# icdm-adteam/MoCoPCI

Measured on AMD Instinct MI355X. Metric: interpolated frames/sec, higher is better.
Workload: dtype f32 (fused MLP layers: fp32 products as 6 bf16-MFMA partials of an exact 3-way split, fp32 accumulate; index paths exact f32)

## Files before the change

mocopci_amd/csrc/knn_cosine.hip:

```cpp
#include "common.h"
#include "topk.h"

namespace {

typedef mcp_key u64;
typedef float f32x16 __attribute__((ext_vector_type(16)));
#define KEY_INF MCP_KEY_INF
constexpr int K = 16, QS = 16, CHK = 4, RT = 32, WAVES = 4;

__device__ __forceinline__ int chan_of(int r, int h) { return (r & 3) + 8 * (r >> 2) + 4 * h; }

template <int C>
__global__ __launch_bounds__(256) void normalize_rows_kernel(long long rows_a, const float *__restrict__ xa, float *__restrict__ ya,
                                                             long long rows_b, const float *__restrict__ xb, float *__restrict__ yb) {
    constexpr int RW = C <= 64 ? 64 : (C == 128 ? 32 : 16), S = C + 1, V = RW * C / 4;
    __shared__ float tile[4][RW * S];
    __shared__ float den[4][RW];
    const int lane = threadIdx.x & 63, wave = threadIdx.x >> 6;
    float *t = tile[wave];
    const long long ta = (rows_a + RW - 1) / RW, tb = (rows_b + RW - 1) / RW;
    for (long long g = (long long)blockIdx.x * 4 + wave; g < ta + tb; g += (long long)gridDim.x * 4) {
        const bool second = g >= ta;
        const float *x = second ? xb : xa;
        float *y = second ? yb : ya;
        const long long rows = second ? rows_b : rows_a, r0 = (second ? g - ta : g) * RW;
        const int live = (int)min((long long)RW, rows - r0);
        const float4 *src = reinterpret_cast<const float4 *>(x + r0 * C);
        __builtin_amdgcn_wave_barrier();
        for (int e = lane; e < V; e += 64) {
            const int row = (e * 4) / C, col = (e * 4) % C;
            if (row < live) {
                const float4 v = src[e];
                float *d = t + row * S + col;
                d[0] = v.x; d[1] = v.y; d[2] = v.z; d[3] = v.w;
            }
        }
        __builtin_amdgcn_wave_barrier();
        if (lane < live) {
            const float *xr = t + lane * S;
            float s = 0.f;
            for (int j = 0; j < C; ++j) s = s + xr[j] * xr[j];
            den[wave][lane] = sqrtf(s + 1e-8f);
        }
        __builtin_amdgcn_wave_barrier();
        float4 *dst = reinterpret_cast<float4 *>(y + r0 * C);
        for (int e = lane; e < V; e += 64) {
            const int row = (e * 4) / C, col = (e * 4) % C;
            if (row < live) {
                const float *d = t + row * S + col;
                const float dn = den[wave][row];
                dst[e] = make_float4(d[0] / dn, d[1] / dn, d[2] / dn, d[3] / dn);
            }
        }
    }
}

template <int C>
void launch_normalize(long long rows_a, const float *xa, float *ya, long long rows_b, const float *xb, float *yb, hipStream_t s) {
    constexpr int RW = C <= 64 ? 64 : (C == 128 ? 32 : 16);
    const long long tiles = (rows_a + RW - 1) / RW + (rows_b + RW - 1) / RW, blocks = (tiles + 3) / 4;
    hipLaunchKernelGGL(normalize_rows_kernel<C>, dim3((unsigned)min(blocks, 4096LL)), dim3(256), 0, s, rows_a, xa, ya, rows_b, xb, yb);
}

template <int C>
__global__ __launch_bounds__(64 * WAVES) void knn_cosine_kernel(int q, int n, int kout, const float *__restrict__ nq,
                                                                const float *__restrict__ nr, int *__restrict__ idx,
                                                                float *__restrict__ dist) {
    constexpr int S = C + 1;
    constexpr int PER_THREAD = RT * C / (64 * WAVES);
    extern __shared__ __attribute__((aligned(16))) float smem[];
    float *tiles = smem;
    const int tid = threadIdx.x, lane = tid & 63, wave = tid >> 6, h = lane >> 5, col = lane & 31;
    uint2(*queue)[64] = reinterpret_cast<uint2(*)[64]>(smem + 2 * RT * S) + (size_t)wave * QS;

    const int b = blockIdx.y;
    const int qi = blockIdx.x * (32 * WAVES) + wave * 32 + col;
    const bool live = qi < q;
    const float *qrow = nq + ((size_t)b * q + (live ? qi : 0)) * C;
    float bq[C / 2];
#pragma unroll
    for (int s = 0; s < C / 2; ++s) bq[s] = qrow[2 * s + h];
    nr += (size_t)b * n * C;

    u64 a[K];
#pragma unroll
    for (int j = 0; j < K; ++j) a[j] = KEY_INF;
    float tau = INFINITY;
    int cnt = 0;
    auto flush = [&]() {
        mcp_flush_queue<K, QS>(a, queue, lane, cnt);
        tau = mcp_tau_of(a[K - 1]);
        cnt = 0;
    };

    const int ntiles = (n + RT - 1) / RT;
    float pre[PER_THREAD];
    auto fetch = [&](int t) {
#pragma unroll
        for (int u = 0; u < PER_THREAD; ++u) {
            const int e = tid + u * 64 * WAVES, row = e / C, cc = e % C;
            const int gr = t * RT + row;
            pre[u] = gr < n ? nr[(size_t)gr * C + cc] : 0.f;
        }
    };
    auto stash = [&](int buf) {
#pragma unroll
        for (int u = 0; u < PER_THREAD; ++u) {
            const int e = tid + u * 64 * WAVES, row = e / C, cc = e % C;
            tiles[buf * RT * S + row * S + cc] = pre[u];
        }
    };
    fetch(0);
    stash(0);
    for (int t = 0; t < ntiles; ++t) {
        const int cur = t & 1;
        if (t + 1 < ntiles) fetch(t + 1);
        __syncthreads();
        const float *ta = tiles + cur * RT * S + col * S + h;
        f32x16 acc;
#pragma unroll
        for (int r = 0; r < 16; ++r) acc[r] = 0.f;
#pragma unroll
        for (int s = 0; s < C / 2; ++s) acc = __builtin_amdgcn_mfma_f32_32x32x2f32(ta[2 * s], bq[s], acc, 0, 0, 0);
        const int base = t * RT;
#pragma unroll
        for (int r0 = 0; r0 < 16; r0 += CHK) {
#pragma unroll
            for (int r = r0; r < r0 + CHK; ++r) {
                const int ri = base + chan_of(r, h);
                const float d = 1.0f - acc[r];
                if (ri < n && d < tau) {
                    queue[cnt][lane] = make_uint2(__float_as_uint(d), (uint32_t)ri);
                    ++cnt;
                }
            }
            if (__builtin_amdgcn_ballot_w64(cnt > QS - CHK)) flush();
        }
        if (t + 1 < ntiles) stash(cur ^ 1);
    }
    flush();
    u64 o[K];
#pragma unroll
    for (int j = 0; j < K; ++j) {
        const uint32_t lo = __shfl_xor(mcp_key_lo(a[j]), 32), hi = __shfl_xor(mcp_key_hi(a[j]), 32);
        o[j] = mcp_key_words(hi, lo);
    }
    mcp_merge_sorted<K, K>(a, o);
    if (!live || h) return;
    int *oi = idx + ((size_t)b * q + qi) * kout;
    float *od = dist ? dist + ((size_t)b * q + qi) * kout : nullptr;
    mcp_store_list<K>(a, kout, oi, od);
}

template <int C, int RS>
__global__ __launch_bounds__(64 * RS) void knn_cosine_split_kernel(int q, int n, int kout, const float *__restrict__ nq,
                                                                   const float *__restrict__ nr, int *__restrict__ idx,
                                                                   float *__restrict__ dist) {
    constexpr int CH = C / 32;
    extern __shared__ __attribute__((aligned(16))) float smem[];
    const int tid = threadIdx.x, lane = tid & 63, wave = tid >> 6, h = lane >> 5, col = lane & 31;
    uint2(*queue)[64] = reinterpret_cast<uint2(*)[64]>(smem) + (size_t)wave * QS;

    const int b = blockIdx.y;
    const int qi = blockIdx.x * 32 + col;
    const bool live = qi < q;
    const float *qrow = nq + ((size_t)b * q + (live ? qi : 0)) * C;
    constexpr bool QL = C > 128;
    float bq[QL ? 1 : C / 2];
    float *ql = smem + (size_t)RS * QS * 64 * 2;
    if (QL) {
        for (int i = wave; i < C / 2; i += RS) ql[i * 64 + lane] = qrow[2 * i + h];
        __syncthreads();
    } else {
#pragma unroll
        for (int j = 0; j < (QL ? 0 : C / 4); ++j) {
            const float4 v = reinterpret_cast<const float4 *>(qrow)[j];
            bq[QL ? 0 : 2 * j] = h ? v.y : v.x;
            bq[QL ? 0 : 2 * j + 1] = h ? v.w : v.z;
        }
    }
    nr += (size_t)b * n * C;

    u64 a[K];
#pragma unroll
    for (int j = 0; j < K; ++j) a[j] = KEY_INF;
    float tau = INFINITY;
    int cnt = 0;
    auto flush = [&]() {
        mcp_flush_queue<K, QS>(a, queue, lane, cnt);
        tau = mcp_tau_of(a[K - 1]);
        cnt = 0;
    };

    const int ntiles = (n + RT - 1) / RT;
    const int mine = wave < ntiles ? (ntiles - wave + RS - 1) / RS : 0;
    auto load = [&](int t, int c, float4 (&v)[8]) {
        const int row = min(t * RT + col, n - 1);
        const float4 *p = reinterpret_cast<const float4 *>(nr + (size_t)row * C + c * 32);
#pragma unroll
        for (int j = 0; j < 8; ++j) v[j] = p[j];
    };
    f32x16 acc;
    auto mfma16 = [&](int c, const float4 (&v)[8]) {
#pragma unroll
        for (int j = 0; j < 8; ++j) {
            const float q0 = QL ? ql[(c * 16 + 2 * j) * 64 + lane] : bq[QL ? 0 : c * 16 + 2 * j];
            const float q1 = QL ? ql[(c * 16 + 2 * j + 1) * 64 + lane] : bq[QL ? 0 : c * 16 + 2 * j + 1];
            acc = __builtin_amdgcn_mfma_f32_32x32x2f32(h ? v[j].y : v[j].x, q0, acc, 0, 0, 0);
            acc = __builtin_amdgcn_mfma_f32_32x32x2f32(h ? v[j].w : v[j].z, q1, acc, 0, 0, 0);
        }
    };
    float4 va[8], vb[8];
    if (mine > 0) load(wave, 0, va);
    for (int ti = 0; ti < mine; ++ti) {
        const int t = wave + ti * RS;
#pragma unroll
        for (int r = 0; r < 16; ++r) acc[r] = 0.f;
#pragma unroll
        for (int c = 0; c < CH; c += 2) {
            load(t, c + 1, vb);
            mfma16(c, va);
            if (c + 2 < CH) load(t, c + 2, va);
            else if (ti + 1 < mine) load(t + RS, 0, va);
            mfma16(c + 1, vb);
        }
        const int base = t * RT;
#pragma unroll
        for (int r0 = 0; r0 < 16; r0 += CHK) {
#pragma unroll
            for (int r = r0; r < r0 + CHK; ++r) {
                const int ri = base + chan_of(r, h);
                const float d = 1.0f - acc[r];
                if (ri < n && d < tau) {
                    queue[cnt][lane] = make_uint2(__float_as_uint(d), (uint32_t)ri);
                    ++cnt;
                }
            }
            if (__builtin_amdgcn_ballot_w64(cnt > QS - CHK)) flush();
        }
    }
    flush();
    u64 o[K];
#pragma unroll
    for (int j = 0; j < K; ++j) {
        const uint32_t lo = __shfl_xor(mcp_key_lo(a[j]), 32), hi = __shfl_xor(mcp_key_hi(a[j]), 32);
        o[j] = mcp_key_words(hi, lo);
    }
    mcp_merge_sorted<K, K>(a, o);
    __syncthreads();
    if (wave > 0 && h == 0) {
#pragma unroll
        for (int j = 0; j < K; ++j) queue[j][col] = make_uint2(mcp_key_lo(a[j]), mcp_key_hi(a[j]));
    }
    __syncthreads();
    if (wave != 0 || h) return;
    for (int w = 1; w < RS; ++w) {
        uint2(*other)[64] = reinterpret_cast<uint2(*)[64]>(smem) + (size_t)w * QS;
#pragma unroll
        for (int j = 0; j < K; ++j) {
            const uint2 e = other[j][col];
            o[j] = mcp_key_words(e.y, e.x);
        }
        mcp_merge_sorted<K, K>(a, o);
    }
    if (!live) return;
    int *oi = idx + ((size_t)b * q + qi) * kout;
    float *od = dist ? dist + ((size_t)b * q + qi) * kout : nullptr;
    mcp_store_list<K>(a, kout, oi, od);
}

template <int C, int RS>
int launch_cosine_split(int b, int q, int n, int k, const float *nq, const float *nr, int *idx, float *dist, hipStream_t s) {
    static_assert(K == QS && (C / 32) % 2 == 0, "the partial lists reuse the queues; chunks are consumed in pairs");
    const size_t lds = (size_t)RS * QS * 64 * sizeof(uint2) + (C > 128 ? (size_t)(C / 2) * 64 * sizeof(float) : 0);
    auto kern = knn_cosine_split_kernel<C, RS>;
    static McpPerDeviceOnce attr_once;
    if (attr_once.need()) {
        { const hipError_t attr_e_ = hipFuncSetAttribute(reinterpret_cast<const void *>(kern), hipFuncAttributeMaxDynamicSharedMemorySize, 160 * 1024); if (attr_e_ != hipSuccess) return (int)attr_e_; }
        attr_once.done();
    }
    hipLaunchKernelGGL(kern, dim3(mcp_divup(q, 32), b), dim3(64 * RS), lds, s, q, n, k, nq, nr, idx, dist);
    return mcp_launch_status();
}

template <int C>
int launch_cosine_auto(int b, int q, int n, int k, const float *nq, const float *nr, int *idx, float *dist, hipStream_t s) {
    const long long groups = (long long)b * ((q + 31) / 32);
    const int tiles = (n + RT - 1) / RT;
    if (groups * 2 >= 2048 || tiles < 4) return launch_cosine_split<C, 2>(b, q, n, k, nq, nr, idx, dist, s);
    if (groups * 4 >= 2048 || tiles < 8) return launch_cosine_split<C, 4>(b, q, n, k, nq, nr, idx, dist, s);
    return launch_cosine_split<C, 8>(b, q, n, k, nq, nr, idx, dist, s);
}

template <int C>
int launch_cosine(int b, int q, int n, int k, const float *nq, const float *nr, int *idx, float *dist, hipStream_t s) {
    const size_t lds = (size_t)2 * RT * (C + 1) * sizeof(float) + (size_t)WAVES * QS * 64 * sizeof(uint2);
    auto kern = knn_cosine_kernel<C>;
    static McpPerDeviceOnce attr_once;
    if (attr_once.need()) {
        { const hipError_t attr_e_ = hipFuncSetAttribute(reinterpret_cast<const void *>(kern), hipFuncAttributeMaxDynamicSharedMemorySize, 160 * 1024); if (attr_e_ != hipSuccess) return (int)attr_e_; }
        attr_once.done();
    }
    hipLaunchKernelGGL(kern, dim3(mcp_divup(q, 32 * WAVES), b), dim3(64 * WAVES), lds, s, q, n, k, nq, nr, idx, dist);
    return mcp_launch_status();
}

}

#ifdef MCP_AB
static int g_cosine_use_old = 0;
extern "C" __attribute__((visibility("default"))) void mcp_knn_cosine_use_old(int on) { g_cosine_use_old = on; }
#endif

MCP_EXPORT int mcp_knn_cosine(int b, int q, int n, int c, int k, const float *qfeat, const float *rfeat, int *idx, float *dist,
                              float *workspace, mcp_stream_t stream) {
    MCP_CHECK_ARGS(b > 0 && q > 0 && n > 0 && c > 0 && k > 0 && qfeat && rfeat && idx && workspace);
    if (k > K || (c != 64 && c != 128 && c != 256)) return MCP_ERR_UNSUPPORTED;
    if ((((uintptr_t)qfeat) | ((uintptr_t)rfeat) | ((uintptr_t)workspace)) & 15) return MCP_ERR_BAD_ARG;
    hipStream_t s = (hipStream_t)stream;
    float *nq = workspace, *nr = workspace + (size_t)b * q * c;
    mcp_prof_begin(MCP_KERNEL_KNN_COSINE, s);
    const long long rq = (long long)b * q, rr = (long long)b * n;
    if (c == 64) launch_normalize<64>(rq, qfeat, nq, rr, rfeat, nr, s);
    else if (c == 128) launch_normalize<128>(rq, qfeat, nq, rr, rfeat, nr, s);
    else launch_normalize<256>(rq, qfeat, nq, rr, rfeat, nr, s);
    int rc = mcp_launch_status();
    if (rc == MCP_OK) {
#ifdef MCP_AB
        if (g_cosine_use_old)
            rc = c == 64    ? launch_cosine<64>(b, q, n, k, nq, nr, idx, dist, s)
                 : c == 128 ? launch_cosine<128>(b, q, n, k, nq, nr, idx, dist, s)
                            : launch_cosine<256>(b, q, n, k, nq, nr, idx, dist, s);
        else
#endif
        rc = c == 64    ? launch_cosine_auto<64>(b, q, n, k, nq, nr, idx, dist, s)
             : c == 128 ? launch_cosine_auto<128>(b, q, n, k, nq, nr, idx, dist, s)
                        : launch_cosine_auto<256>(b, q, n, k, nq, nr, idx, dist, s);
    }
    mcp_prof_end(MCP_KERNEL_KNN_COSINE, s);
    return rc;
}
```

Before: 3672.

## Add tiled cosine KNN kernel sharing reference tiles across query waves

Adds a new cosine KNN kernel in which several query waves (QG) share LDS-staged reference tiles, split into 64-channel chunks and double-buffered with register prefetch. Reference rows are split across RP wave partitions whose partial top-k lists are merged by a binary tree through LDS. The default auto path now launches this kernel with an XCD-aware unit mapping, and the previous split kernel stays available under A/B flags. The intent is to cut redundant global reads of reference features and improve latency hiding. In exchange it adds block-wide syncs per chunk and an LDS merge stage, and lowers the number of reference partitions, which may reduce parallelism on small batches.

```diff
diff --git a/mocopci_amd/csrc/knn_cosine.hip b/mocopci_amd/csrc/knn_cosine.hip
--- a/mocopci_amd/csrc/knn_cosine.hip
+++ b/mocopci_amd/csrc/knn_cosine.hip
@@ -284,12 +284,180 @@
 }
 
 template <int C>
-int launch_cosine_auto(int b, int q, int n, int k, const float *nq, const float *nr, int *idx, float *dist, hipStream_t s) {
+int launch_cosine_split_auto(int b, int q, int n, int k, const float *nq, const float *nr, int *idx, float *dist, hipStream_t s) {
     const long long groups = (long long)b * ((q + 31) / 32);
     const int tiles = (n + RT - 1) / RT;
     if (groups * 2 >= 2048 || tiles < 4) return launch_cosine_split<C, 2>(b, q, n, k, nq, nr, idx, dist, s);
     if (groups * 4 >= 2048 || tiles < 8) return launch_cosine_split<C, 4>(b, q, n, k, nq, nr, idx, dist, s);
     return launch_cosine_split<C, 8>(b, q, n, k, nq, nr, idx, dist, s);
+}
+
+template <int C, int QG, int RP>
+__global__ __launch_bounds__(64 * QG * RP) void knn_cosine_tiles_kernel(int nb, int q, int n, int kout, const float *__restrict__ nq,
+                                                                        const float *__restrict__ nr, int *__restrict__ idx,
+                                                                        float *__restrict__ dist) {
+    constexpr int CW = 64, S = CW + 1, NCH = C / CW;
+    constexpr int WV = QG * RP, PT = 64 * QG;
+    constexpr int V4 = RT * (CW / 4) / PT;
+    constexpr bool QL = C > 128;
+    static_assert(RT * (CW / 4) % PT == 0 && (RP & (RP - 1)) == 0, "whole float4s per thread; the tail is a binary tree");
+    extern __shared__ __attribute__((aligned(16))) float smem[];
+    const int tid = threadIdx.x, lane = tid & 63, wave = tid >> 6, h = lane >> 5, col = lane & 31;
+    const int g = wave % QG, part = wave / QG, ptid = tid - part * PT;
+    uint2(*queue)[64] = reinterpret_cast<uint2(*)[64]>(smem) + (size_t)wave * QS;
+    float *tile = smem + (size_t)WV * QS * 64 * 2 + (size_t)part * 2 * RT * S;
+    float *ql = smem + (size_t)WV * QS * 64 * 2 + (size_t)RP * 2 * RT * S + (size_t)g * (C / 2) * 64;
+
+    const int qblocks = (q + 32 * QG - 1) / (32 * QG);
+    const McpUnits unit = mcp_units_by_xcd((long long)nb * qblocks, 1);
+    if (unit.first >= unit.limit) return;
+    const int b = (int)((uint32_t)unit.first / (uint32_t)qblocks), qb = (int)((uint32_t)unit.first % (uint32_t)qblocks);
+    const int q0 = qb * (32 * QG) + g * 32, qi = q0 + col;
+    const bool live = qi < q, wave_live = q0 < q;
+    const float *qrow = nq + ((size_t)b * q + (live ? qi : 0)) * C;
+    float bq[QL ? 1 : C / 2];
+    if (QL) {
+        for (int j = part; j < C / 4; j += RP) {
+            const float4 v = reinterpret_cast<const float4 *>(qrow)[j];
+            ql[(2 * j) * 64 + lane] = h ? v.y : v.x;
+            ql[(2 * j + 1) * 64 + lane] = h ? v.w : v.z;
+        }
+    } else {
+#pragma unroll
+        for (int j = 0; j < (QL ? 0 : C / 4); ++j) {
+            const float4 v = reinterpret_cast<const float4 *>(qrow)[j];
+            bq[QL ? 0 : 2 * j] = h ? v.y : v.x;
+            bq[QL ? 0 : 2 * j + 1] = h ? v.w : v.z;
+        }
+    }
+    nr += (size_t)b * n * C;
+
+    u64 a[K];
+#pragma unroll
+    for (int j = 0; j < K; ++j) a[j] = KEY_INF;
+    float tau = INFINITY;
+    int cnt = 0;
+    auto flush = [&]() {
+        mcp_flush_queue<K, QS>(a, queue, lane, cnt);
+        tau = mcp_tau_of(a[K - 1]);
+        cnt = 0;
+    };
+
+    const int ntiles = (n + RT - 1) / RT;
+    const int rounds = (ntiles + RP - 1) / RP, nsteps = rounds * NCH;
+    const int mine = part < ntiles ? (ntiles - part + RP - 1) / RP : 0;
+    float4 pre[V4];
+    auto fetch = [&](int st) {
+        const int t = part + (st / NCH) * RP, ch = st % NCH;
+#pragma unroll
+        for (int u = 0; u < V4; ++u) {
+            const int e = ptid + u * PT, row = e / (CW / 4), c4 = e % (CW / 4);
+            const int gr = t * RT + row;
+            pre[u] = gr < n ? *reinterpret_cast<const float4 *>(nr + (size_t)gr * C + ch * CW + c4 * 4) : make_float4(0.f, 0.f, 0.f, 0.f);
+        }
+    };
+    auto stash = [&](int buf) {
+#pragma unroll
+        for (int u = 0; u < V4; ++u) {
+            const int e = ptid + u * PT, row = e / (CW / 4), c4 = e % (CW / 4);
+            float *d = tile + buf * RT * S + row * S + c4 * 4;
+            d[0] = pre[u].x; d[1] = pre[u].y; d[2] = pre[u].z; d[3] = pre[u].w;
+        }
+    };
+    f32x16 acc;
+    fetch(0);
+    stash(0);
+    for (int ti = 0; ti < rounds; ++ti) {
+        const bool work = wave_live && ti < mine;
+#pragma unroll
+        for (int ch = 0; ch < NCH; ++ch) {
+            const int st = ti * NCH + ch, cur = st & 1;
+            if (st + 1 < nsteps) fetch(st + 1);
+            __syncthreads();
+            if (work) {
+                const float *ta = tile + cur * RT * S + col * S + h;
+                if (ch == 0) {
+#pragma unroll
+                    for (int r = 0; r < 16; ++r) acc[r] = 0.f;
+                }
+#pragma unroll
+                for (int s = 0; s < CW / 2; ++s) {
+                    const float qv = QL ? ql[(ch * (CW / 2) + s) * 64 + lane] : bq[QL ? 0 : ch * (CW / 2) + s];
+                    acc = __builtin_amdgcn_mfma_f32_32x32x2f32(ta[2 * s], qv, acc, 0, 0, 0);
+                }
+                if (ch == NCH - 1) {
+                    const int base = (part + ti * RP) * RT;
+#pragma unroll
+                    for (int r0 = 0; r0 < 16; r0 += CHK) {
+#pragma unroll
+                        for (int r = r0; r < r0 + CHK; ++r) {
+                            const int ri = base + chan_of(r, h);
+                            const float d = 1.0f - acc[r];
+                            if (ri < n && d < tau) {
+                                queue[cnt][lane] = make_uint2(__float_as_uint(d), (uint32_t)ri);
+                                ++cnt;
+                            }
+                        }
+                        if (__builtin_amdgcn_ballot_w64(cnt > QS - CHK)) flush();
+                    }
+                }
+            }
+            if (st + 1 < nsteps) stash(cur ^ 1);
+        }
+    }
+    flush();
+    u64 o[K];
+#pragma unroll
+    for (int j = 0; j < K; ++j) {
+        const uint32_t lo = __shfl_xor(mcp_key_lo(a[j]), 32), hi = __shfl_xor(mcp_key_hi(a[j]), 32);
+        o[j] = mcp_key_words(hi, lo);
+    }
+    mcp_merge_sorted<K, K>(a, o);
+#pragma unroll
+    for (int s = 1; s < RP; s <<= 1) {
+        if ((part & (2 * s - 1)) == s && h == 0) {
+#pragma unroll
+            for (int j = 0; j < K; ++j) queue[j][col] = make_uint2(mcp_key_lo(a[j]), mcp_key_hi(a[j]));
+        }
+        __syncthreads();
+        if ((part & (2 * s - 1)) == 0) {
+            uint2(*other)[64] = reinterpret_cast<uint2(*)[64]>(smem) + (size_t)(wave + s * QG) * QS;
+#pragma unroll
+            for (int j = 0; j < K; ++j) {
+                const uint2 e = other[j][col];
+                o[j] = mcp_key_words(e.y, e.x);
+            }
+            mcp_merge_sorted<K, K>(a, o);
+        }
+    }
+    if (part != 0 || h || !live) return;
+    int *oi = idx + ((size_t)b * q + qi) * kout;
+    float *od = dist ? dist + ((size_t)b * q + qi) * kout : nullptr;
+    mcp_store_list<K>(a, kout, oi, od);
+}
+
+template <int C, int QG, int RP>
+int launch_cosine_tiles(int b, int q, int n, int k, const float *nq, const float *nr, int *idx, float *dist, hipStream_t s) {
+    static_assert(K == QS, "the partial lists reuse the queues");
+    constexpr size_t lds = ((size_t)QG * RP * QS * 64 * 2 + (size_t)RP * 2 * RT * 65 + (C > 128 ? (size_t)QG * (C / 2) * 64 : 0)) * sizeof(float);
+    static_assert(lds <= 160 * 1024, "one workgroup's LDS");
+    const long long units = (long long)b * ((q + 32 * QG - 1) / (32 * QG));
+    if (units > 0x7FFFFFF0LL) return MCP_ERR_UNSUPPORTED;
+    auto kern = knn_cosine_tiles_kernel<C, QG, RP>;
+    static McpPerDeviceOnce attr_once;
+    if (attr_once.need()) {
+        { const hipError_t attr_e_ = hipFuncSetAttribute(reinterpret_cast<const void *>(kern), hipFuncAttributeMaxDynamicSharedMemorySize, 160 * 1024); if (attr_e_ != hipSuccess) return (int)attr_e_; }
+        attr_once.done();
+    }
+    hipLaunchKernelGGL(kern, dim3((unsigned)((units + 7) / 8 * 8)), dim3(64 * QG * RP), lds, s, b, q, n, k, nq, nr, idx, dist);
+    return mcp_launch_status();
+}
+
+template <int C>
+int launch_cosine_auto(int b, int q, int n, int k, const float *nq, const float *nr, int *idx, float *dist, hipStream_t s) {
+    constexpr int QG = C > 128 ? 2 : 4;
+    if (n <= RT) return launch_cosine_tiles<C, QG, 1>(b, q, n, k, nq, nr, idx, dist, s);
+    return launch_cosine_tiles<C, QG, 2>(b, q, n, k, nq, nr, idx, dist, s);
 }
 
 template <int C>
@@ -327,7 +495,15 @@
     int rc = mcp_launch_status();
     if (rc == MCP_OK) {
 #ifdef MCP_AB
-        if (g_cosine_use_old)
+        if (g_cosine_use_old == 3)
+            rc = c == 64    ? launch_cosine_tiles<64, 2, 4>(b, q, n, k, nq, nr, idx, dist, s)
+                 : c == 128 ? launch_cosine_tiles<128, 2, 4>(b, q, n, k, nq, nr, idx, dist, s)
+                            : launch_cosine_tiles<256, 2, 2>(b, q, n, k, nq, nr, idx, dist, s);
+        else if (g_cosine_use_old == 2)
+            rc = c == 64    ? launch_cosine_split_auto<64>(b, q, n, k, nq, nr, idx, dist, s)
+                 : c == 128 ? launch_cosine_split_auto<128>(b, q, n, k, nq, nr, idx, dist, s)
+                            : launch_cosine_split_auto<256>(b, q, n, k, nq, nr, idx, dist, s);
+        else if (g_cosine_use_old)
             rc = c == 64    ? launch_cosine<64>(b, q, n, k, nq, nr, idx, dist, s)
                  : c == 128 ? launch_cosine<128>(b, q, n, k, nq, nr, idx, dist, s)
                             : launch_cosine<256>(b, q, n, k, nq, nr, idx, dist, s);
```

After: 3636. No clear change (-1.0%).
